# philres/ngmlr

Measured on AMD Instinct MI355X. Metric: aligned Gbp/hour (PacBio 10kb synthetic, convex-gap SW hot path, host buffers in -> results out, CIGAR bit-exact), higher is better.
Workload: dtype f32

## Files before the change

### ngmlr_amd/csrc/cvx_kernels.hip

```cpp
#include <hip/hip_runtime.h>
#include <stdint.h>

#include "cvx_types.h"
#include "cvx_launch.h"

namespace cvx {

#define CVX_DEV __device__ __forceinline__

CVX_DEV int rot1_i(int v) {
	return __builtin_amdgcn_update_dpp(0, v, 0x13C, 0xf, 0xf, true);
}
CVX_DEV float rot1_f(float v) {
	return __int_as_float(rot1_i(__float_as_int(v)));
}


CVX_DEV void row_span(const int2 ol, int W, int y, int &gs, int &ge) {
	long long lo = ol.x > 0 ? ol.x : 0;
	long long hi = (long long) ol.x + (long long) ol.y;
	if (hi > W) hi = W;
	if (hi < lo) hi = lo;
	gs = (int) (lo + y);
	ge = (int) (hi + y);
// ... 848 lines not shown
		for (int j = 0; j < M; ++j) { d[2 * j] = sh ? accA[j] << sh : accA[j]; d[2 * j + 1] = sh ? accB[j] << sh : accB[j]; }
	}

	float b = -1.0f;
	int by = 0x7fffffff, bx = 0x7fffffff;
#pragma unroll
	for (int j = 0; j < M; ++j) {
		int vy = s_besty[j][tid];
		const int ycur = (int) (ref_base - (xa[j] - (unsigned) r - 4u));
		if (ycur < H && best_r[j] >= r - cnt[j]) vy = ycur;
		const float v = best[j];
		const int vx = best_r[j] - vy;
		if (v > 0.0f) {
			if (v > b || (v == b && (vy < by || (vy == by && vx < bx)))) { b = v; by = vy; bx = vx; }
		}
	}
	float be = lbest;
#pragma unroll
	for (int off = 32; off >= 1; off >>= 1) {
		const float ob = __shfl_xor(b, off, 64);
		const int oy = __shfl_xor(by, off, 64);
		const int ox = __shfl_xor(bx, off, 64);
		if (ob > b || (ob == b && (oy < by || (oy == by && ox < bx)))) { b = ob; by = oy; bx = ox; }
		if (!EXACT) be = fmaxf(be, __shfl_xor(be, off, 64));
	}
	if (CHAIN) {
		if (lane == 0) {
			ChainOut co;
			co.score = b;
			co.best_y = (b > -1.0f) ? by + y0 : 0;
			co.best_x = (b > -1.0f) ? bx - y0 : 0;
			co.failed = chain_failed;
			a.chain_out[ct.blk] = co;
			unsigned long long *ticks = reinterpret_cast<unsigned long long *>(a.redo_count + kCtrChainTicks);
			atomicAdd(ticks, (unsigned long long) (__builtin_amdgcn_s_memtime() - chain_t0));
			if (chain_polled) atomicAdd(ticks + 1, (unsigned long long) chain_polled);
		}
		return;
	}
	if (GANG) {
		if (lane == 0) {
			s_gred[wv][0] = b; s_gred[wv][1] = __int_as_float(by); s_gred[wv][2] = __int_as_float(bx);
			s_gred[wv][3] = EXACT ? 0.0f : be;
			s_gfail[wv] = gang_failed;
		}
		__syncthreads();
		if (wv != 0) return;
#pragma unroll
		for (int w = 1; w < G; ++w) {
			const float ob = s_gred[w][0];
			const int oy = __float_as_int(s_gred[w][1]), ox = __float_as_int(s_gred[w][2]);
			if (ob > b || (ob == b && (oy < by || (oy == by && ox < bx)))) { b = ob; by = oy; bx = ox; }
			if (!EXACT) be = fmaxf(be, s_gred[w][3]);
		}
	}
	if (lane == 0) {
		TileOut o;
		o.score = b;
		o.status = 0;
		o.best_x = (b > -1.0f) ? bx : 0;
		o.best_y = (b > -1.0f) ? by : 0;
		o.ref_position = 0; o.qstart = 0; o.qend = 0; o.n_ops = 0; o.ops_first = 0;
		o.pad = (!EXACT && gswitch > 0 && !(b > be + 2.0f * a.sp.mat + 1.0f)) ? kPadRedo : 0;
		if (GANG) {
			bool failed = gang_failed != 0;
			for (int w = 1; w < G; ++w) failed = failed || s_gfail[w] != 0;
			if (failed) { o.status = -1; o.pad = 0; }
		}
		a.tout[t] = o;
	}
}

CVX_DEV int rec_load(const void *rec, const int n_dwords, const int lane) {
	return lane < n_dwords ? reinterpret_cast<const int *>(rec)[lane] : 0;
}
CVX_DEV int fld(const int w, const int k) { return __builtin_amdgcn_readlane(w, k); }
CVX_DEV unsigned long long fld64(const int w, const int k) {
	return ((unsigned long long) (unsigned) fld(w, k + 1) << 32) | (unsigned) fld(w, k);
}

CVX_DEV void walk_tile(const BacktrackArgs &a, const int t, const int lane) {
	static_assert(sizeof(TileRun) == 48 && sizeof(TileIn) == 32 && sizeof(TileOut) == 40, "record layout");
	const int wr = rec_load(a.trun + t, 12, lane);
	const int wo = rec_load(a.tout + t, 10, lane);
	if (fld(wr, 8) != 0) return;
	TileOut o;
	o.score = __int_as_float(fld(wo, 0));
	o.status = fld(wo, 1);
	o.best_x = fld(wo, 2); o.best_y = fld(wo, 3);
	o.ref_position = 0; o.qstart = 0; o.qend = 0; o.n_ops = 0; o.ops_first = 0;
	o.pad = fld(wo, 9);
	if (o.status != 0 || o.pad != 0) return;
	const int wi = rec_load(a.tin + t, 8, lane);
	const int H = fld(wi, 3), W = fld(wi, 2);
	const RowView rows = row_view(a.rsrc[t], a.rows, fld64(wi, 4));
	if (!(o.score > 0.0f)) {
		int fy, fx;
		first_cell(rows, H, W, lane, &fy, &fx);
		if (fy < 0) {
			o.score = -1.0f; o.status = 5; o.pad = 1;
			if (lane == 0) a.tout[t] = o;
			return;
		}
		o.score = 0.0f; o.best_x = fx; o.best_y = fy;
	}
	const int cb0 = fld(wr, 10);
	if (cb0 >= 0)
		backtrack_walk<true>(lane, H, fld(wr, 4), fld(wr, 6), fld(wr, 5), rows,
				reinterpret_cast<const uint2 *>(a.dirs), a.chain_blk + cb0,
				a.seq + (unsigned) fld(wi, 0), a.seq + (unsigned) fld(wi, 1),
				a.ops + fld64(wr, 2), o);
	else
		backtrack_walk<false>(lane, H, fld(wr, 4), fld(wr, 6), fld(wr, 5), rows,
				reinterpret_cast<const uint2 *>(a.dirs + fld64(wr, 0)), nullptr,
				a.seq + (unsigned) fld(wi, 0), a.seq + (unsigned) fld(wi, 1),
				a.ops + fld64(wr, 2), o);
	o.pad = 1;
	if (lane == 0) a.tout[t] = o;
}


template <int G>
struct Group {
	int gl;
	int base;
	CVX_DEV unsigned ballot(bool p) const {
		const u64 b = __builtin_amdgcn_ballot_w64(p);
		return (unsigned) (b >> base) & (G == 32 ? 0xffffffffu : ((1u << (G & 31)) - 1u));
	}
	CVX_DEV int bcast(int v, int l) const { return __shfl(v, base + l, 64); }
};

template <int G>
CVX_DEV void backtrack_walk_grp(const Group<G> g, const bool has_tile, const bool chained, const int H, const int N, const int r0, const int ops_cap,
		const RowView &rows, const uint2 *dirs, const ChainBlk *blk, const uint8_t *ref, const uint8_t *qry, int *ops, TileOut &o) {
	const int gl = g.gl;
	const int best_x = o.best_x, best_y = o.best_y;
	bool act = has_tile;
	if (has_tile && best_y <= 0) { o.status = 1; act = false; }
	const bool walked = act;

	const int qend = (H - best_y) - 1;
	int idx = ops_cap - 1;
	int elem = 4;
	int elem_len = qend;
	int consumed = qend;
	int x = best_x, y = best_y;
	int s = act ? y % N : 0;
	int status = 0;
	unsigned want = 3u;
	int budget = 2 * (best_x + best_y) + 8;

	auto emit = [&](int cur, int n) {
		if (n <= 0) return;
		if (cur == elem) {
			elem_len += n;
		} else {
			if (elem != 4) { if (gl == 0) ops[idx] = (elem_len << 4) | elem; idx -= 1; }
			elem = cur;
			elem_len = n;
		}
	};
	int c_gb = -1;
	ChainBlk c_cb;
	c_cb.dir_off = 0; c_cb.tblk0 = 0; c_cb.nblk32 = 1;

	while (__builtin_amdgcn_ballot_w64(act) != 0ull) {
		if (act) {
			bool go_on = true;
			if (--budget < 0) { status = 3; go_on = false; }
			else {
				const int dx = (want != 1u) ? 1 : 0, dy = (want != 2u) ? 1 : 0;
				const int cx = x - gl * dx, cy = y - gl * dy;
				const bool inside = (cx >= 0 && cy >= 0);
				const int lx = cx > 0 ? cx : 0, ly = cy > 0 ? cy : 0;
				int sl = s - gl * dy;
				if (sl < 0) sl += N;
				const int tt = cx + cy - r0;
				const int ttc = tt > 0 ? tt : 0;
				const RowDesc2 ol = row_at(rows, ly);
				size_t widx = (size_t) (ttc >> 5) * N + sl;
				if (chained) {
					const int gb = ly / N;
					if (gb != c_gb) { c_cb = blk[gb]; c_gb = gb; }
					int wr = (ttc >> 5) - c_cb.tblk0;
					wr = wr < 0 ? 0 : (wr >= c_cb.nblk32 ? c_cb.nblk32 - 1 : wr);
					widx = c_cb.dir_off + (size_t) wr * N + (size_t) (ly - gb * N);
				}
				const uint2 w = dirs[widx];
				const int rc = ref[lx], qc = qry[ly];
				const unsigned eqm = g.ballot(rc == qc);
				const bool in_row = inside && tt >= 0 && cx >= ol.x && cx < ol.x + ol.y;
				unsigned code = plane_code(w.x, w.y, 31 - (ttc & 31));
				if (!in_row) code = 0u;
				int minC, maxC;
				valid_bounds(ol.x, ol.y, minC, maxC);

				const unsigned full = (G == 32) ? 0xffffffffu : ((1u << (G & 31)) - 1u);
				const unsigned run = g.ballot(code == want);
				const int L = (run == full) ? G : __builtin_ctz(~run);
				const unsigned low = (L == G) ? full : ((1u << L) - 1u);
				const unsigned vp = g.ballot(cx > minC && cx < maxC);
				if ((~vp & low) != 0u) { status = 2; go_on = false; }
				else {
					if (want == 3u) {
						if (L > 0) {
							const unsigned e = eqm & low;
							const unsigned starts = (((e ^ (e << 1)) & low) & ~1u) | 1u;
							const int k = __builtin_popcount(starts);
							const int op0 = (e & 1u) ? 7 : 8;
							if (k == 1) {
								emit(op0, L);
							} else {
								const unsigned after0 = starts & ~1u;
								int len0 = __builtin_ctz(after0);
								int w0 = 0;
								if (op0 == elem) len0 += elem_len;
								else if (elem != 4) { if (gl == 0) ops[idx] = (elem_len << 4) | elem; w0 = 1; }
								const bool is_start = gl < L && ((starts >> gl) & 1u) != 0u;
								const int j = __builtin_popcount(starts & ((1u << gl) - 1u));
								const unsigned rest = (starts >> gl) >> 1;
								int mylen = rest ? __builtin_ctz(rest) + 1 : L - gl;
								if (gl == 0) mylen = len0;
								const int myop = ((e >> gl) & 1u) ? 7 : 8;
								if (is_start && j < k - 1) ops[idx - w0 - j] = (mylen << 4) | myop;
								idx -= w0 + (k - 1);
								const int lastpos = 31 - __builtin_clz(starts);
								elem = ((e >> lastpos) & 1u) ? 7 : 8;
								elem_len = L - lastpos;
							}
						}
						x -= L; y -= L; consumed += L;
					} else if (want == 1u) {
						emit(1, L);
						y -= L; consumed += L;
					} else {
						emit(2, L);
						x -= L;
					}
					if (want != 2u) { s -= L; if (s < 0) s += N; }
					if (L < G) {
						const unsigned nxt = (unsigned) g.bcast((int) code, L);
						if (nxt == 0u) go_on = false;
						else if (want != 3u) want = nxt;
						else {
							const int tp = x + y - r0;
							if (nxt == 2u) {
								const unsigned wx = (unsigned) g.bcast((int) w.x, L);
								const unsigned wy = (unsigned) g.bcast((int) w.y, L);
								const int row_lo = max(g.bcast(ol.x, L), 0);
								const int b0 = 31 - (tp & 31);
								const unsigned dm = (wx & ~wy) >> b0;
								int Ld = (~dm == 0u) ? 32 : __builtin_ctz(~dm);
								const int in_word = 32 - b0;
								const int in_rowc = x - row_lo + 1;
								if (Ld > in_rowc) Ld = in_rowc;
								const int rminC = g.bcast(minC, L), rmaxC = g.bcast(maxC, L);
								if (!(x - (Ld - 1) > rminC && x < rmaxC)) { status = 2; go_on = false; }
								else {
									emit(2, Ld);
									x -= Ld;
									if (Ld == in_rowc) go_on = false;
									else if (Ld == in_word) want = 2u;
									else {
										const unsigned c2 = plane_code(wx, wy, b0 + Ld);
										if (c2 == 0u) go_on = false; else want = c2;
									}
								}
							} else {
								const int k = gl - L;
								const int tn = tp - k;
								const bool have = (k >= 0) && (cy >= 0) && (tn >= 0) && ((tn >> 5) == (ttc >> 5));
								const bool col_in = (x >= ol.x) && (x < ol.x + ol.y);
								unsigned c2 = plane_code(w.x, w.y, 31 - (tn & 31));
								if (!col_in) c2 = 0u;
								const unsigned im = g.ballot(have && c2 == 1u) >> L;
								const int Li = (~im == 0u) ? 32 : __builtin_ctz(~im);
								const unsigned ilow = (Li >= 32) ? 0xffffffffu : ((1u << Li) - 1u);
								const unsigned vpi = g.ballot(x > minC && x < maxC) >> L;
								if ((~vpi & ilow) != 0u) { status = 2; go_on = false; }
								else {
									emit(1, Li);
									y -= Li; consumed += Li;
									s -= Li; if (s < 0) s += N;
									const int en = L + Li;
									want = 1u;
									const unsigned hv = g.ballot(have);
									const int c3i = g.bcast((int) c2, en < G ? en : 0);
									if (en < G && ((hv >> en) & 1u) != 0u) {
										if (c3i == 0) go_on = false; else want = (unsigned) c3i;
									}
								}
							}
						}
					}
				}
			}
			if (!go_on) act = false;
		}
	}
	if (walked) {
		if (status == 0) {
			if (elem != 4) { if (gl == 0) ops[idx] = (elem_len << 4) | elem; idx -= 1; }
			consumed += (y + 1);
			o.ref_position = x + 1;
			o.qstart = y + 1;
			o.qend = qend;
			o.ops_first = idx + 1;
			o.n_ops = ops_cap - 1 - idx;
			if (H != consumed) status = 3;
		}
		o.status = status;
	}
}

template <int G>
__global__ void __launch_bounds__(64)
backtrack_grp_kernel(const BacktrackArgs a, const int32_t *order, const int n_order) {
	const int lane = threadIdx.x;
	Group<G> g;
	g.gl = lane & (G - 1);
	g.base = lane & ~(G - 1);
	const int q = blockIdx.x * (64 / G) + lane / G;
	bool has = q < n_order;
	const int t = has ? order[q] : 0;
	TileOut o;
	o.score = -1.0f; o.status = 0; o.best_x = 0; o.best_y = 0;
	o.ref_position = 0; o.qstart = 0; o.qend = 0; o.n_ops = 0; o.ops_first = 0; o.pad = 0;
	TileRun tr;
	TileIn ti;
	tr.skip = 1; tr.ring = 64; tr.r0 = 0; tr.ops_cap = 8; tr.dir_off = 0; tr.ops_off = 0; tr.chain_blk0 = -1;
	ti.H = 0; ti.W = 0; ti.row_off = 0; ti.ref_off = 0; ti.qry_off = 0;
	if (has) {
		tr = a.trun[t];
		o = a.tout[t];
		ti = a.tin[t];
		if (tr.skip != 0 || o.status != 0 || o.pad != 0) has = false;
	}
	const int H = ti.H, W = ti.W;
	const RowView rows = row_view(a.rsrc[t], a.rows, ti.row_off);
	bool dead = false;
	if (__builtin_amdgcn_ballot_w64(has && !(o.score > 0.0f)) != 0ull) {
		if (has && !(o.score > 0.0f)) {
			int fy = -1, fx = 0;
			bool searching = true;
			for (int y0 = 0; __builtin_amdgcn_ballot_w64(searching && y0 < H) != 0ull; y0 += G) {
				if (searching && y0 < H) {
					const int yy = y0 + g.gl;
					bool hc = false;
					int lo_i = 0;
					if (yy < H) {
						const RowDesc2 ol = row_at(rows, yy);
						long long lo = ol.x > 0 ? ol.x : 0;
						long long hi = (long long) ol.x + (long long) ol.y;
						if (hi > W) hi = W;
						hc = hi > lo;
						lo_i = (int) lo;
					}
					const unsigned m = g.ballot(hc);
					const int l = m ? __builtin_ctz(m) : 0;
					const int fxl = g.bcast(lo_i, l);
					if (m != 0u) { fy = y0 + l; fx = fxl; searching = false; }
				}
			}
			if (fy < 0) { dead = true; has = false; }
			else { o.score = 0.0f; o.best_x = fx; o.best_y = fy; }
		}
	}
	const bool chained = tr.chain_blk0 >= 0;
	int *ops = a.ops + tr.ops_off;
	const uint8_t *ref = a.seq + ti.ref_off, *qry = a.seq + ti.qry_off;
	const uint2 *dirs = reinterpret_cast<const uint2 *>(chained ? a.dirs : a.dirs + tr.dir_off);
	backtrack_walk_grp<G>(g, has, chained, H, tr.ring, tr.r0, tr.ops_cap, rows, dirs,
			a.chain_blk + (chained ? tr.chain_blk0 : 0), ref, qry, ops, o);
	if (dead) { o.score = -1.0f; o.status = 5; }
	if ((has || dead) && g.gl == 0) { o.pad = 1; a.tout[t] = o; }
}

__global__ void __launch_bounds__(64)
backtrack_kernel(const BacktrackArgs a, const int32_t *order, const int n_order) {
	if ((int) blockIdx.x >= n_order) return;
	const int t = order ? order[blockIdx.x] : (int) blockIdx.x;
	walk_tile(a, t, threadIdx.x);
}

__global__ void __launch_bounds__(256)
finalize_kernel(const TileOut *tout, const TilePlan *plan, uint64_t *dst_off, ResultRec *res,
		BatchSummary *sum, int32_t *counters, int n_tiles, unsigned long long dense_cap) {
	constexpr int T = 256;
	__shared__ unsigned long long s_part[T];
	const int tid = threadIdx.x;
	const int per = (n_tiles + T - 1) / T;
	const int t0 = min(n_tiles, tid * per), t1 = min(n_tiles, t0 + per);
	unsigned long long mine = 0;
	for (int t = t0; t < t1; ++t) {
		const TileOut o = tout[t];
		if (o.status == 0 && o.n_ops > 0) mine += (unsigned long long) o.n_ops;
	}
	s_part[tid] = mine;
	__syncthreads();
	for (int d = 1; d < T; d <<= 1) {
		const unsigned long long v = (tid >= d) ? s_part[tid - d] : 0ull;
		__syncthreads();
		s_part[tid] += v;
		__syncthreads();
	}
	unsigned long long off = s_part[tid] - mine;
	int n_valid = 0;
	for (int t = t0; t < t1; ++t) {
		const TileOut o = tout[t];
		ResultRec r;
		r.score = o.score;
		r.status = o.status;
		r.best_x = o.best_x; r.best_y = o.best_y;
		r.ref_position = o.ref_position; r.qstart = o.qstart; r.qend = o.qend;
		r.n_ops = (o.status == 0) ? o.n_ops : 0;
		r.ops_begin = off;
		r.cells = plan[t].cells;
		res[t] = r;
		dst_off[t] = off;
		if (o.status == 0) { n_valid += 1; if (o.n_ops > 0) off += (unsigned long long) o.n_ops; }
	}
	__shared__ int s_valid;
	if (tid == 0) s_valid = 0;
	__syncthreads();
	if (n_valid) atomicAdd(&s_valid, n_valid);
	__syncthreads();
	if (tid == T - 1) {
		BatchSummary b;
		b.ops_total = s_part[T - 1];
		b.dense_cap = dense_cap;
		b.n_valid = s_valid;
		b.n_redone = counters ? counters[0] : 0;
		b.chain_task_ticks = counters ? reinterpret_cast<const unsigned long long *>(counters + kCtrChainTicks)[0] : 0ull;
		b.chain_poll_ticks = counters ? reinterpret_cast<const unsigned long long *>(counters + kCtrChainTicks)[1] : 0ull;
		*sum = b;
	}
	__syncthreads();
	if (counters && tid < 64) counters[tid] = 0;
}

__global__ void __launch_bounds__(256)
compact_ops_kernel(const int32_t *regions, const TileRun *trun, const TileOut *tout,
		const uint64_t *dst_off, uint32_t *dense, int n_tiles, unsigned long long dense_cap) {
	const int t = blockIdx.x;
	if (t >= n_tiles) return;
	const TileOut o = tout[t];
	if (o.status != 0 || o.n_ops <= 0) return;
	const unsigned long long d0 = dst_off[t];
	if (d0 + (unsigned long long) o.n_ops > dense_cap) return;
	const int32_t *src = regions + trun[t].ops_off + o.ops_first;
	uint32_t *dst = dense + d0;
	for (int i = threadIdx.x; i < o.n_ops; i += blockDim.x) dst[i] = (uint32_t) src[i];
}


__global__ void __launch_bounds__(64)
chain_reduce_kernel(const int32_t *tiles, int n_tiles, const TileRun *trun, const ChainOut *cout, TileOut *tout) {
	const int q = blockIdx.x;
	if (q >= n_tiles) return;
	const int t = tiles[q];
	const TileRun tr = trun[t];
	const int lane = threadIdx.x;
	float b = -1.0f;
	int by = 0x7fffffff, bx = 0x7fffffff, failed = 0;
	for (int g = lane; g < tr.chain_nblk; g += 64) {
		const ChainOut c = cout[tr.chain_blk0 + g];
		failed |= c.failed;
		if (c.score > b) { b = c.score; by = c.best_y; bx = c.best_x; }
	}
#pragma unroll
	for (int off = 32; off >= 1; off >>= 1) {
		const float ob = __shfl_xor(b, off, 64);
		const int oy = __shfl_xor(by, off, 64);
		const int ox = __shfl_xor(bx, off, 64);
		failed |= __shfl_xor(failed, off, 64);
		if (ob > b || (ob == b && (oy < by || (oy == by && ox < bx)))) { b = ob; by = oy; bx = ox; }
	}
	if (lane == 0) {
		TileOut o;
		o.score = b;
		o.status = failed ? -1 : 0;
		o.best_x = (b > -1.0f) ? bx : 0;
		o.best_y = (b > -1.0f) ? by : 0;
		o.ref_position = 0; o.qstart = 0; o.qend = 0; o.n_ops = 0; o.ops_first = 0;
		o.pad = 0;
		tout[t] = o;
	}
}

template <int G>
static hipError_t launch_fill_gang(const FillArgs &a, int mode, hipStream_t st) {
	if (mode == kFillExact) hipLaunchKernelGGL((fill_ring_kernel<3, false, kFillExact, false, G>), dim3(a.list_n), dim3(64 * G), 0, st, a);
	else if (a.pen_table) hipLaunchKernelGGL((fill_ring_kernel<3, false, kFillTwoPhase, true, G>), dim3(a.list_n), dim3(64 * G), 0, st, a);
	else hipLaunchKernelGGL((fill_ring_kernel<3, false, kFillTwoPhase, false, G>), dim3(a.list_n), dim3(64 * G), 0, st, a);
	return hipGetLastError();
}

template <int M, bool WRAP>
static hipError_t launch_fill_t(const FillArgs &a, int mode, size_t pad_lds, hipStream_t st) {
	if (mode == kFillChain) {
		if constexpr (M == 1 || M == 2 || M == 4) hipLaunchKernelGGL((fill_ring_kernel<M, WRAP, kFillChain>), dim3(a.list_n), dim3(64), pad_lds, st, a);
		else return hipErrorInvalidValue;
	} else if (mode == kFillExact) hipLaunchKernelGGL((fill_ring_kernel<M, WRAP, kFillExact>), dim3(a.list_n), dim3(64), 0, st, a);
	else if (!WRAP && a.pen_table) hipLaunchKernelGGL((fill_ring_kernel<M, false, kFillTwoPhase, true>), dim3(a.list_n), dim3(64), 0, st, a);
	else hipLaunchKernelGGL((fill_ring_kernel<M, WRAP, kFillTwoPhase>), dim3(a.list_n), dim3(64), 0, st, a);
	return hipGetLastError();
}

template <int M>
static hipError_t launch_fill_w(const FillArgs &a, bool wrap, int mode, size_t pad_lds, hipStream_t st) {
	return wrap ? launch_fill_t<M, true>(a, mode, pad_lds, st) : launch_fill_t<M, false>(a, mode, pad_lds, st);
}

hipError_t launch_fill(int m, int gang, bool wrap, int mode, const FillArgs &a, size_t pad_lds, hipStream_t st) {
	if (a.list_n <= 0) return hipSuccess;
	if (gang > 1) {
		if (m != 3 || wrap || mode == kFillChain) return hipErrorInvalidValue;
		return gang == 2 ? launch_fill_gang<2>(a, mode, st) : gang == 3 ? launch_fill_gang<3>(a, mode, st) : hipErrorInvalidValue;
	}
	switch (m) {
	case 1: return launch_fill_w<1>(a, wrap, mode, pad_lds, st);
	case 2: return launch_fill_w<2>(a, wrap, mode, pad_lds, st);
	case 3: return launch_fill_w<3>(a, wrap, mode, pad_lds, st);
	case 4: return launch_fill_w<4>(a, wrap, mode, pad_lds, st);
	default: return hipErrorInvalidValue;
	}
}

hipError_t launch_chain_reduce(const int32_t *tiles, int n_tiles, const TileRun *trun, const ChainOut *cout, TileOut *tout, hipStream_t st) {
	if (n_tiles <= 0) return hipSuccess;
	hipLaunchKernelGGL(chain_reduce_kernel, dim3(n_tiles), dim3(64), 0, st, tiles, n_tiles, trun, cout, tout);
	return hipGetLastError();
}

hipError_t launch_expand_rows(const RowSrc *rsrc, const TileIn *tin, const uint8_t *delta, const RowDesc *rowsx, RowDesc *rows,
		int n_tiles, bool closed_forms, hipStream_t st) {
	if (n_tiles <= 0) return hipSuccess;
	hipLaunchKernelGGL(expand_rows_kernel, dim3(n_tiles), dim3(64), 0, st, rsrc, tin, delta,
			reinterpret_cast<const int2 *>(rowsx), reinterpret_cast<int2 *>(rows), n_tiles, closed_forms ? 1 : 0);
	return hipGetLastError();
}

hipError_t launch_plan(const RowDesc *rows, const RowSrc *rsrc, const TileIn *tin, TilePlan *plan, int n_tiles, uint64_t rows_per_tile,
		unsigned long long max_matrix_mb, hipStream_t st) {
	if (n_tiles <= 0) return hipSuccess;
	if (rows_per_tile >= 1024)
		hipLaunchKernelGGL(plan_kernel<256>, dim3(n_tiles), dim3(256), 0, st,
				reinterpret_cast<const int2 *>(rows), rsrc, tin, plan, n_tiles, max_matrix_mb);
	else
		hipLaunchKernelGGL(plan_kernel<64>, dim3((n_tiles + 3) / 4), dim3(256), 0, st,
				reinterpret_cast<const int2 *>(rows), rsrc, tin, plan, n_tiles, max_matrix_mb);
	return hipGetLastError();
}

hipError_t launch_backtrack(const BacktrackArgs &a, const int32_t *order, int n_order, int group, hipStream_t st) {
	if (a.n_tiles <= 0) return hipSuccess;
	if (group == 16 && order != nullptr) {
		if (n_order <= 0) return hipSuccess;
		hipLaunchKernelGGL(backtrack_grp_kernel<16>, dim3((n_order + 3) / 4), dim3(64), 0, st, a, order, n_order);
	} else if (group == 4 && order != nullptr) {
		if (n_order <= 0) return hipSuccess;
		hipLaunchKernelGGL(backtrack_grp_kernel<4>, dim3((n_order + 15) / 16), dim3(64), 0, st, a, order, n_order);
	} else if (group == 8 && order != nullptr) {
		if (n_order <= 0) return hipSuccess;
		hipLaunchKernelGGL(backtrack_grp_kernel<8>, dim3((n_order + 7) / 8), dim3(64), 0, st, a, order, n_order);
	} else if (group == 32 && order != nullptr) {
		if (n_order <= 0) return hipSuccess;
		hipLaunchKernelGGL(backtrack_grp_kernel<32>, dim3((n_order + 1) / 2), dim3(64), 0, st, a, order, n_order);
	} else {
		const int nb = order != nullptr ? n_order : a.n_tiles;
		if (nb <= 0) return hipSuccess;
		hipLaunchKernelGGL(backtrack_kernel, dim3(nb), dim3(64), 0, st, a, order, nb);
	}
	return hipGetLastError();
}

hipError_t launch_finalize(const TileOut *tout, const TilePlan *plan, uint64_t *dst_off, ResultRec *res,
		BatchSummary *sum, int32_t *counters, int n_tiles, uint64_t dense_cap, hipStream_t st) {
	hipLaunchKernelGGL(finalize_kernel, dim3(1), dim3(256), 0, st, tout, plan, dst_off, res, sum, counters,
			n_tiles, (unsigned long long) dense_cap);
	return hipGetLastError();
}

hipError_t launch_compact(const int32_t *regions, const TileRun *trun, const TileOut *tout,
		const uint64_t *dst_off, uint32_t *dense, int n_tiles, uint64_t dense_cap, hipStream_t st) {
	if (n_tiles <= 0) return hipSuccess;
	hipLaunchKernelGGL(compact_ops_kernel, dim3(n_tiles), dim3(256), 0, st, regions, trun, tout, dst_off, dense, n_tiles,
			(unsigned long long) dense_cap);
	return hipGetLastError();
}

}
```

### ngmlr_amd/csrc/cvx_launch.h

```cpp
#ifndef CVX_LAUNCH_H
#define CVX_LAUNCH_H

#include <hip/hip_runtime_api.h>
#include <stdint.h>

#include "cvx_types.h"

namespace cvx {

hipError_t launch_fill(int m, int gang, bool wrap, int mode, const FillArgs &a, size_t pad_lds, hipStream_t st);
hipError_t launch_chain_reduce(const int32_t *tiles, int n_tiles, const TileRun *trun, const ChainOut *cout, TileOut *tout, hipStream_t st);
struct ScorePair {
	uint64_t ref_off, qry_off;
	uint64_t scratch_off;
	int32_t ref_len, qry_len;
};
hipError_t launch_score(const uint8_t *seq, const ScorePair *pairs, int32_t *scratch, float *out, int n, int max_ref_len, hipStream_t st);
hipError_t launch_score_diag(const uint8_t *seq, const ScorePair *pairs, float *out, int n, hipStream_t st);

struct SearchCandidate {
	uint64_t location;
	float score;
	int32_t reverse;
};
struct SearchArgs {
	const uint2 *rows;
	const uint32_t *locs;
	unsigned long long unit_offset;
	int32_t k;
	const uint8_t *seq;
	const uint64_t *seq_off;
	const int32_t *seq_len;
	int32_t n;
	unsigned long long *events;
	const uint64_t *list_off;
	uint32_t *rlist;
	uint32_t *undo;
	SearchCandidate *cand;
	int32_t *n_cand;
	float *max_hit;
	int32_t *kmer_misses;
	const int32_t *work;
	int32_t n_work;
	int32_t bits;
	float hpoc_factor;
	uint64_t *keys;
	float *scores;
	float sensitivity, min_hits;
	int32_t bin_shift;
	const uint64_t *cand_off;
};
static const int kSearchWaveLog2Min = 9, kSearchWaveLog2Max = 12, kSearchWaveLog2Default = 11;
static const int kSearchWaveSeq = 4096;
static inline int search_wave_entries(const int log2s) { return (3 << log2s) / 4; }
static inline int search_wave_log2(const unsigned long long votes) {
	for (int l = kSearchWaveLog2Min; l < kSearchWaveLog2Max; ++l) if (votes <= (unsigned long long) search_wave_entries(l)) return l;
	return kSearchWaveLog2Max;
}
static const int kSearchNeedsHbm = -2;
size_t search_wave_lds_bytes(int log2s, int seq_cap, bool slot8);
hipError_t launch_search_count(const SearchArgs &a, hipStream_t st);
hipError_t launch_search(const SearchArgs &a, hipStream_t st);
hipError_t launch_search_wave(const SearchArgs &a, int log2s, int seq_cap, bool slot8, hipStream_t st);
hipError_t launch_search_wave_hbm(const SearchArgs &a, int n_tables, unsigned int *ticket, hipStream_t st);
hipError_t launch_search_compact(const SearchCandidate *sparse, const uint64_t *src_off, const int32_t *n_cand, const uint64_t *dst_begin,
		SearchCandidate *dense, int n, hipStream_t st);

hipError_t launch_decode_windows(const uint8_t *bin, const uint64_t *starts, int n_starts,
		const WindowDesc *win, int n, uint8_t *dst, hipStream_t st);

hipError_t launch_text_size(const TextArgs &a, hipStream_t st);
hipError_t launch_text_write(const TextArgs &a, hipStream_t st);
hipError_t launch_nm_offsets(const TextArgs &a, int first, int count, unsigned long long *len, unsigned long long *off, unsigned long long *total, hipStream_t st);
hipError_t launch_nm_profile(const TextArgs &a, int first, int count, const unsigned long long *off, int32_t *triples, hipStream_t st);

size_t generic_scratch_bytes(int ring);
hipError_t launch_fill_generic(const FillArgs &a, bool sse_variant, uint8_t *scratch, const uint64_t *scratch_off, hipStream_t st);
hipError_t launch_expand_rows(const RowSrc *rsrc, const TileIn *tin, const uint8_t *delta, const RowDesc *rowsx, RowDesc *rows,
		int n_tiles, bool closed_forms, hipStream_t st);
hipError_t launch_plan(const RowDesc *rows, const RowSrc *rsrc, const TileIn *tin, TilePlan *plan, int n_tiles, uint64_t rows_per_tile,
		unsigned long long max_matrix_mb, hipStream_t st);
hipError_t launch_backtrack(const BacktrackArgs &a, const int32_t *order, int n_order, int group, hipStream_t st);
hipError_t launch_finalize(const TileOut *tout, const TilePlan *plan, uint64_t *dst_off, ResultRec *res,
		BatchSummary *sum, int32_t *counters, int n_tiles, uint64_t dense_cap, hipStream_t st);
hipError_t launch_compact(const int32_t *regions, const TileRun *trun, const TileOut *tout,
		const uint64_t *dst_off, uint32_t *dense, int n_tiles, uint64_t dense_cap, hipStream_t st);

}
#endif
```

### ngmlr_amd/csrc/cvx_rt_align.cpp

```cpp
#include <algorithm>
#include <atomic>
#include <chrono>
#include <cstdio>
#include <cstdlib>
#include <cstring>
#include <new>
#include <string>
#include <vector>

#include "cvx_rt.h"

namespace {

static const size_t kPoolBatches = 8;

cvx_batch_s *acquire_batch(cvx_context *h) {
	if (!h->pool.empty()) {
		cvx_batch_s *b = h->pool.back();
		h->pool.pop_back();
		return b;
	}
	return new (std::nothrow) cvx_batch_s();
}

void recycle_batch(cvx_context *h, cvx_batch_s *b) {
	const bool failed = b->state == kFailed;
	b->state = kEmpty;
	b->in_flight = false;
	b->have_ops = false;
	b->have_refs = false;
	b->text_done = false;
	b->fail_rc = CVX_OK;
	b->fail_msg.clear();
	if (h) {
		auto it = std::find(h->live.begin(), h->live.end(), b);
		if (it != h->live.end()) h->live.erase(it);
	}
	if (h && !failed && h->pool.size() < kPoolBatches) { h->pool.push_back(b); return; }
	b->release();
	delete b;
}

void discard_batch(cvx_context *h, cvx_batch_s *b) {
	(void) hipDeviceSynchronize();
	if (h) {
		auto it = std::find(h->pending.begin(), h->pending.end(), b);
		if (it != h->pending.end()) h->pending.erase(it);
		it = std::find(h->live.begin(), h->live.end(), b);
		if (it != h->live.end()) h->live.erase(it);
	}
	b->release();
	delete b;
}

int fail_job(cvx_batch_s *b, int rc) {
	(void) hipDeviceSynchronize();
	b->state = kFailed;
	b->fail_rc = rc;
	b->fail_msg = g_err;
	return rc;
}

int stage_upload(cvx_context *h, cvx_batch_s *b, int32_t n, const cvx_tile *tiles,
		const cvx_genome_s *genome = nullptr, const uint64_t *ref_position = nullptr) {
	RC_TRY(ensure_streams(h));
	UploadLayout L;
	std::vector<TileIn> tin;
	int bad = -1;
	const bool windows = genome != nullptr;
	const int lrc = upload_layout(n, tiles, tin, L, &bad, windows);
	if (lrc == kLayoutMalformed) { set_err("tile %d malformed", bad); return CVX_ERR_ARG; }
	if (lrc == kLayoutTooLarge) {
		set_err("%llu sequence bytes exceed one batch (4 GiB); split the batch", (unsigned long long) L.seq_total);
		return CVX_ERR_ARG;
	}
	b->n = n;
	b->state = kEmpty;
	b->have_ops = false;
	b->have_refs = false;
	b->text_done = false;
	b->ops_total = 0;
	b->seq_total = L.seq_total;
	b->n_rows = L.n_rows;
	memset(&b->timing, 0, sizeof(b->timing));
	RC_TRY(b->make_events());
	const size_t n1 = (size_t) std::max(n, 1);
	const size_t rows1 = (size_t) std::max<uint64_t>(L.arena_rows, 1);
	RC_TRY(b->h_delta.ensure((size_t) L.delta_total + 256));
	RC_TRY(b->h_rsrc.ensure(n1 * sizeof(RowSrc)));
	RC_TRY(b->d_delta.ensure((size_t) L.delta_total + 256));
	RC_TRY(b->d_rsrc.ensure(n1));
	RC_TRY(b->h_tin.ensure(n1 * sizeof(TileIn)));
	RC_TRY(b->h_plan.ensure(n1 * sizeof(TilePlan)));
	RC_TRY(b->h_res.ensure(n1 * sizeof(ResultRec) + sizeof(BatchSummary)));
	RC_TRY(b->d_seq.ensure((size_t) L.seq_total + 256));
	RC_TRY(b->d_rows.ensure(rows1));
	RC_TRY(b->d_tin.ensure(n1));
	RC_TRY(b->d_plan.ensure(n1));
	RC_TRY(b->d_trun.ensure(n1));
	RC_TRY(b->d_tout.ensure(n1));
	RC_TRY(b->d_dstoff.ensure(n1));
	RC_TRY(b->d_lists.ensure(2 * n1));
	if (b->d_counters.cap < 64) {
		RC_TRY(b->d_counters.ensure(64));
		HIP_TRY(hipMemset(b->d_counters.p, 0, b->d_counters.cap * sizeof(int32_t)));
	}
	RC_TRY(b->d_res.ensure(n1 * sizeof(ResultRec) + sizeof(BatchSummary)));
	if (n) memcpy(b->h_tin.p, tin.data(), (size_t) n * sizeof(TileIn));

	const bool zc_qry = n > 0 && L.qry_contig && L.qry_bytes > 0 && in_pinned_block(tiles[0].qry, L.qry_bytes + 4);
	const bool zc_ref = n > 0 && !windows && L.ref_contig && L.ref_bytes > 0 && in_pinned_block(tiles[0].ref, L.ref_bytes + 4);
	b->zero_copy_bytes = (zc_qry ? L.qry_bytes : 0) + (zc_ref ? L.ref_bytes : 0);
	const bool pack_seq = !(zc_qry && (zc_ref || windows));
	if (pack_seq) RC_TRY(b->h_seq.ensure((size_t) L.seq_total + 256));
	uint8_t *hseq = b->h_seq.as<uint8_t>();
	uint8_t *hdelta = b->h_delta.as<uint8_t>();
	std::vector<RowOverflow> overflow;
	hipStream_t st = h->s_io;
	if (pack_seq) upload_zero_pads(L, hseq);
	if (zc_qry || zc_ref) {
		const uint64_t zmax = L.pad + 1024;
		RC_TRY(b->h_zero.ensure((size_t) zmax));
		if (b->zero_cap != b->h_zero.cap) { memset(b->h_zero.p, 0, b->h_zero.cap); b->zero_cap = b->h_zero.cap; }
		auto zero_range = [&](uint64_t lo, uint64_t hi) -> int {
			lo = lo / 256 * 256;
			hi = std::min<uint64_t>((hi + 255) / 256 * 256, (L.seq_total + 255) / 256 * 256);
			for (uint64_t at = lo; at < hi; at += zmax / 256 * 256) {
				const uint64_t len = std::min<uint64_t>(hi - at, zmax / 256 * 256);
				HIP_TRY(hipMemcpyAsync(b->d_seq.p + at, b->h_zero.p, (size_t) len, hipMemcpyHostToDevice, st));
			}
			return CVX_OK;
		};
		if (zc_qry) {
			RC_TRY(zero_range(0, L.qry_base));
			RC_TRY(zero_range(L.qry_base + L.qry_bytes, L.ref_base));
			HIP_TRY(hipMemcpyAsync(b->d_seq.p + L.qry_base, tiles[0].qry, (size_t) ((L.qry_bytes + 3) / 4 * 4), hipMemcpyHostToDevice, st));
		}
		if (zc_ref) {
			RC_TRY(zero_range(L.ref_base + L.ref_bytes, L.seq_total));
			HIP_TRY(hipMemcpyAsync(b->d_seq.p + L.ref_base, tiles[0].ref, (size_t) ((L.ref_bytes + 3) / 4 * 4), hipMemcpyHostToDevice, st));
		}
	}
	uint64_t pack_work = L.delta_total * 9ull;
	if (!zc_qry) pack_work += L.qry_bytes;
	if (!zc_ref && !windows) pack_work += L.ref_bytes;
	const std::vector<uint64_t> &wprefix = L.wprefix;
	int threads = std::max(1, std::min(h->pack_threads, PackPool::get().size()));
	if (pack_work < (8u << 20)) threads = 1;
	const int pieces = threads > 1 ? 8 : 1;
	int t0 = 0;
	uint64_t a_done = 0, b_done = L.ref_base, delta_done = 0;
	const uint64_t a_end_all = L.ref_base, b_end_all = (L.seq_total + 255) / 256 * 256;
	for (int pc = 1; pc <= pieces; ++pc) {
		int t1 = n;
		if (pc < pieces) {
			const uint64_t target = wprefix[(size_t) n] / (uint64_t) pieces * (uint64_t) pc;
			t1 = (int) (std::upper_bound(wprefix.begin(), wprefix.end(), target) - wprefix.begin());
			t1 = std::min(std::max(t1, t0), n);
		}
		if (t1 > t0 && pack_work > 0) {
			std::vector<uint64_t> wp((size_t) (t1 - t0) + 1);
			for (int i = t0; i <= t1; ++i) wp[(size_t) (i - t0)] = wprefix[(size_t) i] - wprefix[(size_t) t0];
			const int base = t0;
			const size_t first = overflow.size();
			overflow.resize(first + (size_t) threads + 1);
			std::atomic<int> slot(0);
			parallel_ranges(t1 - t0, wp, threads, [&](int bg, int en) {
				upload_pack(base + bg, base + en, tiles, tin, hseq, hdelta, L.rsrc, overflow[first + (size_t) slot.fetch_add(1)], !zc_qry, !zc_ref && !windows);
			});
		}
		if (!zc_qry) {
			const uint64_t a_end = (t1 == n) ? a_end_all : (uint64_t) tin[(size_t) t1].qry_off / 256 * 256;
			if (a_end > a_done) HIP_TRY(hipMemcpyAsync(b->d_seq.p + a_done, hseq + a_done, (size_t) (a_end - a_done), hipMemcpyHostToDevice, st));
			a_done = std::max(a_done, a_end);
		}
		if (!zc_ref && !windows) {
			const uint64_t b_end = (t1 == n) ? b_end_all : (uint64_t) tin[(size_t) t1].ref_off / 256 * 256;
			if (b_end > b_done) HIP_TRY(hipMemcpyAsync(b->d_seq.p + b_done, hseq + b_done, (size_t) (b_end - b_done), hipMemcpyHostToDevice, st));
			b_done = std::max(b_done, b_end);
		}
		if (L.delta_total) {
			uint64_t del_end = L.delta_total;
			if (t1 < n) {
				int q = t1;
				while (q < n && L.rsrc[(size_t) q].fmt != kRowsDelta8 && L.rsrc[(size_t) q].fmt != kRowsExplicit) q++;
				if (q < n) del_end = L.rsrc[(size_t) q].src_off;
			}
			del_end = (t1 == n) ? (del_end + 255) / 256 * 256 : del_end / 256 * 256;
			if (del_end > delta_done)
				HIP_TRY(hipMemcpyAsync(b->d_delta.p + delta_done, hdelta + delta_done, (size_t) (del_end - delta_done), hipMemcpyHostToDevice, st));
			delta_done = std::max(delta_done, del_end);
		}
		t0 = t1;
	}
	if (n) HIP_TRY(hipMemcpyAsync(b->d_tin.p, b->h_tin.p, (size_t) n * sizeof(TileIn), hipMemcpyHostToDevice, st));
	if (n) {
		uint64_t n_x = 0;
		for (const RowOverflow &o : overflow) n_x += o.rows.size();
		b->n_rowsx = n_x;
		if (n_x) {
			RC_TRY(b->h_rowsx.ensure((size_t) n_x * sizeof(RowDesc)));
			RC_TRY(b->d_rowsx.ensure((size_t) n_x));
			RowDesc *hx = b->h_rowsx.as<RowDesc>();
			uint64_t at = 0;
			for (const RowOverflow &o : overflow) {
				uint64_t r = 0;
				for (int32_t ti : o.tiles) {
					L.rsrc[(size_t) ti].src_off = at + r;
					r += (uint64_t) tin[(size_t) ti].H;
				}
				if (!o.rows.empty()) memcpy(hx + at, o.rows.data(), o.rows.size() * sizeof(RowDesc));
				at += o.rows.size();
			}
			HIP_TRY(hipMemcpyAsync(b->d_rowsx.p, hx, (size_t) n_x * sizeof(RowDesc), hipMemcpyHostToDevice, st));
		}
		memcpy(b->h_rsrc.p, L.rsrc.data(), (size_t) n * sizeof(RowSrc));
		HIP_TRY(hipMemcpyAsync(b->d_rsrc.p, b->h_rsrc.p, (size_t) n * sizeof(RowSrc), hipMemcpyHostToDevice, st));
		if (L.arena_rows) HIP_TRY(launch_expand_rows(b->d_rsrc.p, b->d_tin.p, b->d_delta.p, b->d_rowsx.p, b->d_rows.p, n, false, st));
	}
	if (windows && n) {
		RC_TRY(b->h_win.ensure((size_t) n * sizeof(WindowDesc)));
		RC_TRY(b->d_win.ensure((size_t) n));
		WindowDesc *hw = b->h_win.as<WindowDesc>();
		for (int i = 0; i < n; ++i) {
			hw[i].position = ref_position[i];
			hw[i].dst_off = tin[(size_t) i].ref_off;
			hw[i].n_chars = tiles[i].ref_len;
		}
		HIP_TRY(hipMemcpyAsync(b->d_win.p, hw, (size_t) n * sizeof(WindowDesc), hipMemcpyHostToDevice, st));
		HIP_TRY(hipMemsetAsync(b->d_seq.p + L.ref_base + L.ref_bytes, 0, (size_t) (L.seq_total - L.ref_base - L.ref_bytes), st));
		HIP_TRY(launch_decode_windows(genome->d_bin.p, genome->d_starts.p, genome->n_starts, b->d_win.p, n, b->d_seq.p, st));
		RC_TRY(b->h_refs.ensure((size_t) L.ref_bytes + 64));
		HIP_TRY(hipMemcpyAsync(b->h_refs.p, b->d_seq.p + L.ref_base, (size_t) L.ref_bytes, hipMemcpyDeviceToHost, st));
		b->refs_base = L.ref_base;
		b->have_refs = true;
	}
	b->state = kUploaded;
	return CVX_OK;
}

int stage_plan(cvx_context *h, cvx_batch_s *b, hipStream_t st) {
	const int n = b->n;
	HIP_TRY(hipEventRecord(b->ev[0], st));
	if (n) {
		HIP_TRY(launch_plan(b->d_rows.p, b->d_rsrc.p, b->d_tin.p, b->d_plan.p, n, b->n_rows / (uint64_t) n, h->max_matrix_mb, st));
		HIP_TRY(hipMemcpyAsync(b->h_plan.p, b->d_plan.p, (size_t) n * sizeof(TilePlan), hipMemcpyDeviceToHost, st));
	}
	HIP_TRY(hipEventRecord(b->ev[1], st));
	HIP_TRY(hipEventRecord(b->ev_in, st));
	b->state = kPlanned;
	return CVX_OK;
}

int stage_compute(cvx_context *h, cvx_batch_s *b, bool streaming = false) {
// ... 702 lines not shown
```

Measured before the change: 16060.

## Branchless backtrack walk, waves-per-EU hint, and multi-block finalize scan

The backtrack walk loop is restructured so the bounds check is folded into the run ballot, emit becomes branchless, and the gap step is merged into a single deferred position update, which reduces divergence and ballots per step. The backtrack kernel gets an amdgpu_waves_per_eu(6) hint that trades registers for occupancy. The single-block finalize kernel is replaced by a two-pass multi-block prefix sum: per-block partials are stored after dst_off, then each block scans its own tiles. This costs an extra launch and a larger dst_off buffer, and the register cap could cause spills.

```diff
diff --git a/ngmlr_amd/csrc/cvx_kernels.hip b/ngmlr_amd/csrc/cvx_kernels.hip
--- a/ngmlr_amd/csrc/cvx_kernels.hip
+++ b/ngmlr_amd/csrc/cvx_kernels.hip
@@ -1024,24 +1024,24 @@
 	int budget = 2 * (best_x + best_y) + 8;
 
 	auto emit = [&](int cur, int n) {
-		if (n <= 0) return;
-		if (cur == elem) {
-			elem_len += n;
-		} else {
-			if (elem != 4) { if (gl == 0) ops[idx] = (elem_len << 4) | elem; idx -= 1; }
-			elem = cur;
-			elem_len = n;
-		}
+		const bool some = n > 0;
+		const bool same = cur == elem;
+		const bool flush = some && !same && elem != 4;
+		if (flush && gl == 0) ops[idx] = (elem_len << 4) | elem;
+		idx -= flush ? 1 : 0;
+		elem_len = some ? (same ? elem_len + n : n) : elem_len;
+		elem = some ? cur : elem;
 	};
 	int c_gb = -1;
 	ChainBlk c_cb;
 	c_cb.dir_off = 0; c_cb.tblk0 = 0; c_cb.nblk32 = 1;
 
-	while (__builtin_amdgcn_ballot_w64(act) != 0ull) {
+	if (__builtin_amdgcn_ballot_w64(act) != 0ull) do {
 		if (act) {
-			bool go_on = true;
-			if (--budget < 0) { status = 3; go_on = false; }
-			else {
+			const bool spent = --budget < 0;
+			bool go_on = !spent;
+			if (spent) status = 3;
+			{
 				const int dx = (want != 1u) ? 1 : 0, dy = (want != 2u) ? 1 : 0;
 				const int cx = x - gl * dx, cy = y - gl * dy;
 				const bool inside = (cx >= 0 && cy >= 0);
@@ -1069,54 +1069,45 @@
 				valid_bounds(ol.x, ol.y, minC, maxC);
 
 				const unsigned full = (G == 32) ? 0xffffffffu : ((1u << (G & 31)) - 1u);
-				const unsigned run = g.ballot(code == want);
-				const int L = (run == full) ? G : __builtin_ctz(~run);
+				const unsigned run = g.ballot(code == want && cx > minC && cx < maxC);
+				const int Lr = (run == full) ? G : __builtin_ctz(~run);
+				const unsigned nxt = (unsigned) g.bcast((int) code, Lr & (G - 1));
+				const bool rejected = !spent && Lr < G && nxt == want;
+				if (rejected) { status = 2; go_on = false; }
+				const int L = go_on ? Lr : 0;
 				const unsigned low = (L == G) ? full : ((1u << L) - 1u);
-				const unsigned vp = g.ballot(cx > minC && cx < maxC);
-				if ((~vp & low) != 0u) { status = 2; go_on = false; }
-				else {
-					if (want == 3u) {
-						if (L > 0) {
-							const unsigned e = eqm & low;
-							const unsigned starts = (((e ^ (e << 1)) & low) & ~1u) | 1u;
+				{
+					int gap_op = 0, gap_n = 0;
+					const int mx0 = (want != 1u) ? L : 0, my0 = (want != 2u) ? L : 0;
+					int mx = mx0, my = my0;
+					unsigned nwant = want;
+					{
+						const bool diag = want == 3u;
+						const unsigned e = eqm & low;
+						const unsigned starts = (((e ^ (e << 1)) & low) & ~1u) | 1u;
+						const unsigned after0 = diag ? (starts & ~1u) : 0u;
+						emit(diag ? ((e & 1u) ? 7 : 8) : (int) want, (L > 0 && after0 != 0u) ? __builtin_ctz(after0) : L);
+						if (L > 0 && after0 != 0u) {
 							const int k = __builtin_popcount(starts);
-							const int op0 = (e & 1u) ? 7 : 8;
-							if (k == 1) {
-								emit(op0, L);
-							} else {
-								const unsigned after0 = starts & ~1u;
-								int len0 = __builtin_ctz(after0);
-								int w0 = 0;
-								if (op0 == elem) len0 += elem_len;
-								else if (elem != 4) { if (gl == 0) ops[idx] = (elem_len << 4) | elem; w0 = 1; }
-								const bool is_start = gl < L && ((starts >> gl) & 1u) != 0u;
-								const int j = __builtin_popcount(starts & ((1u << gl) - 1u));
-								const unsigned rest = (starts >> gl) >> 1;
-								int mylen = rest ? __builtin_ctz(rest) + 1 : L - gl;
-								if (gl == 0) mylen = len0;
-								const int myop = ((e >> gl) & 1u) ? 7 : 8;
-								if (is_start && j < k - 1) ops[idx - w0 - j] = (mylen << 4) | myop;
-								idx -= w0 + (k - 1);
-								const int lastpos = 31 - __builtin_clz(starts);
-								elem = ((e >> lastpos) & 1u) ? 7 : 8;
-								elem_len = L - lastpos;
-							}
+							const bool is_start = gl < L && ((starts >> gl) & 1u) != 0u;
+							const int j = __builtin_popcount(starts & ((1u << gl) - 1u));
+							const unsigned rest = (starts >> gl) >> 1;
+							int mylen = rest ? __builtin_ctz(rest) + 1 : L - gl;
+							if (gl == 0) mylen = elem_len;
+							const int myop = ((e >> gl) & 1u) ? 7 : 8;
+							if (is_start && j < k - 1) ops[idx - j] = (mylen << 4) | myop;
+							idx -= k - 1;
+							const int lastpos = 31 - __builtin_clz(starts);
+							elem = ((e >> lastpos) & 1u) ? 7 : 8;
+							elem_len = L - lastpos;
 						}
-						x -= L; y -= L; consumed += L;
-					} else if (want == 1u) {
-						emit(1, L);
-						y -= L; consumed += L;
-					} else {
-						emit(2, L);
-						x -= L;
 					}
-					if (want != 2u) { s -= L; if (s < 0) s += N; }
-					if (L < G) {
-						const unsigned nxt = (unsigned) g.bcast((int) code, L);
+					if (go_on && L < G) {
 						if (nxt == 0u) go_on = false;
-						else if (want != 3u) want = nxt;
+						else if (want != 3u) nwant = nxt;
 						else {
-							const int tp = x + y - r0;
+							const int xg = x - mx0, yg = y - my0;
+							const int tp = xg + yg - r0;
 							if (nxt == 2u) {
 								const unsigned wx = (unsigned) g.bcast((int) w.x, L);
 								const unsigned wy = (unsigned) g.bcast((int) w.y, L);
@@ -1125,52 +1116,55 @@
 								const unsigned dm = (wx & ~wy) >> b0;
 								int Ld = (~dm == 0u) ? 32 : __builtin_ctz(~dm);
 								const int in_word = 32 - b0;
-								const int in_rowc = x - row_lo + 1;
+								const int in_rowc = xg - row_lo + 1;
 								if (Ld > in_rowc) Ld = in_rowc;
 								const int rminC = g.bcast(minC, L), rmaxC = g.bcast(maxC, L);
-								if (!(x - (Ld - 1) > rminC && x < rmaxC)) { status = 2; go_on = false; }
+								if (!(xg - (Ld - 1) > rminC && xg < rmaxC)) { status = 2; go_on = false; }
 								else {
-									emit(2, Ld);
-									x -= Ld;
+									gap_op = 2; gap_n = Ld;
+									mx += Ld;
 									if (Ld == in_rowc) go_on = false;
-									else if (Ld == in_word) want = 2u;
+									else if (Ld == in_word) nwant = 2u;
 									else {
 										const unsigned c2 = plane_code(wx, wy, b0 + Ld);
-										if (c2 == 0u) go_on = false; else want = c2;
+										if (c2 == 0u) go_on = false; else nwant = c2;
 									}
 								}
 							} else {
 								const int k = gl - L;
 								const int tn = tp - k;
 								const bool have = (k >= 0) && (cy >= 0) && (tn >= 0) && ((tn >> 5) == (ttc >> 5));
-								const bool col_in = (x >= ol.x) && (x < ol.x + ol.y);
+								const bool col_in = (xg >= ol.x) && (xg < ol.x + ol.y);
 								unsigned c2 = plane_code(w.x, w.y, 31 - (tn & 31));
 								if (!col_in) c2 = 0u;
 								const unsigned im = g.ballot(have && c2 == 1u) >> L;
 								const int Li = (~im == 0u) ? 32 : __builtin_ctz(~im);
 								const unsigned ilow = (Li >= 32) ? 0xffffffffu : ((1u << Li) - 1u);
-								const unsigned vpi = g.ballot(x > minC && x < maxC) >> L;
+								const unsigned vpi = g.ballot(xg > minC && xg < maxC) >> L;
 								if ((~vpi & ilow) != 0u) { status = 2; go_on = false; }
 								else {
-									emit(1, Li);
-									y -= Li; consumed += Li;
-									s -= Li; if (s < 0) s += N;
+									gap_op = 1; gap_n = Li;
+									my += Li;
 									const int en = L + Li;
-									want = 1u;
+									nwant = 1u;
 									const unsigned hv = g.ballot(have);
 									const int c3i = g.bcast((int) c2, en < G ? en : 0);
 									if (en < G && ((hv >> en) & 1u) != 0u) {
-										if (c3i == 0) go_on = false; else want = (unsigned) c3i;
+										if (c3i == 0) go_on = false; else nwant = (unsigned) c3i;
 									}
 								}
 							}
 						}
+						emit(gap_op, gap_n);
 					}
+					x -= mx; y -= my; consumed += my;
+					s -= my; if (s < 0) s += N;
+					want = nwant;
 				}
 			}
 			if (!go_on) act = false;
 		}
-	}
+	} while (__builtin_amdgcn_ballot_w64(act) != 0ull);
 	if (walked) {
 		if (status == 0) {
 			if (elem != 4) { if (gl == 0) ops[idx] = (elem_len << 4) | elem; idx -= 1; }
@@ -1187,7 +1181,7 @@
 }
 
 template <int G>
-__global__ void __launch_bounds__(64)
+__global__ void __launch_bounds__(64) __attribute__((amdgpu_waves_per_eu(6)))
 backtrack_grp_kernel(const BacktrackArgs a, const int32_t *order, const int n_order) {
 	const int lane = threadIdx.x;
 	Group<G> g;
@@ -1256,19 +1250,50 @@
 	walk_tile(a, t, threadIdx.x);
 }
 
-__global__ void __launch_bounds__(256)
-finalize_kernel(const TileOut *tout, const TilePlan *plan, uint64_t *dst_off, ResultRec *res,
+constexpr int kFinalizeThreads = 256;
+
+CVX_DEV unsigned long long block_sum(unsigned long long v, unsigned long long *s_w, const int tid) {
+#pragma unroll
+	for (int off = 32; off >= 1; off >>= 1) v += __shfl_xor(v, off, 64);
+	__syncthreads();
+	if ((tid & 63) == 0) s_w[tid >> 6] = v;
+	__syncthreads();
+	return s_w[0] + s_w[1] + s_w[2] + s_w[3];
+}
+
+__global__ void __launch_bounds__(kFinalizeThreads)
+finalize_sums_kernel(const TileOut *tout, unsigned long long *part, int n_tiles) {
+	__shared__ unsigned long long s_w[kFinalizeThreads / 64];
+	const int tid = threadIdx.x;
+	const int t = blockIdx.x * kFinalizeThreads + tid;
+	unsigned long long mine = 0, valid = 0;
+	if (t < n_tiles) {
+		const TileOut o = tout[t];
+		if (o.status == 0) { valid = 1; if (o.n_ops > 0) mine = (unsigned long long) o.n_ops; }
+	}
+	const unsigned long long ops = block_sum(mine, s_w, tid);
+	const unsigned long long nv = block_sum(valid, s_w, tid);
+	if (tid == 0) { part[2 * blockIdx.x] = ops; part[2 * blockIdx.x + 1] = nv; }
+}
+
+__global__ void __launch_bounds__(kFinalizeThreads)
+finalize_kernel(const TileOut *tout, const TilePlan *plan, uint64_t *dst_off, const unsigned long long *part, ResultRec *res,
 		BatchSummary *sum, int32_t *counters, int n_tiles, unsigned long long dense_cap) {
-	constexpr int T = 256;
+	constexpr int T = kFinalizeThreads;
+	__shared__ unsigned long long s_w[T / 64];
 	__shared__ unsigned long long s_part[T];
 	const int tid = threadIdx.x;
-	const int per = (n_tiles + T - 1) / T;
-	const int t0 = min(n_tiles, tid * per), t1 = min(n_tiles, t0 + per);
-	unsigned long long mine = 0;
-	for (int t = t0; t < t1; ++t) {
-		const TileOut o = tout[t];
-		if (o.status == 0 && o.n_ops > 0) mine += (unsigned long long) o.n_ops;
-	}
+	const int blk = blockIdx.x, n_blk = gridDim.x;
+	const int upto = blk == 0 ? n_blk : blk;
+	unsigned long long before = 0, valid_all = 0;
+	for (int j = tid; j < upto; j += T) { before += part[2 * j]; valid_all += part[2 * j + 1]; }
+	before = block_sum(before, s_w, tid);
+	if (blk == 0) valid_all = block_sum(valid_all, s_w, tid);
+	const int t = blk * T + tid;
+	TileOut o;
+	o.status = -1; o.n_ops = 0;
+	if (t < n_tiles) o = tout[t];
+	const unsigned long long mine = (o.status == 0 && o.n_ops > 0) ? (unsigned long long) o.n_ops : 0ull;
 	s_part[tid] = mine;
 	__syncthreads();
 	for (int d = 1; d < T; d <<= 1) {
@@ -1277,10 +1302,8 @@
 		s_part[tid] += v;
 		__syncthreads();
 	}
-	unsigned long long off = s_part[tid] - mine;
-	int n_valid = 0;
-	for (int t = t0; t < t1; ++t) {
-		const TileOut o = tout[t];
+	if (t < n_tiles) {
+		const unsigned long long off = (blk == 0 ? 0ull : before) + s_part[tid] - mine;
 		ResultRec r;
 		r.score = o.score;
 		r.status = o.status;
@@ -1291,18 +1314,13 @@
 		r.cells = plan[t].cells;
 		res[t] = r;
 		dst_off[t] = off;
-		if (o.status == 0) { n_valid += 1; if (o.n_ops > 0) off += (unsigned long long) o.n_ops; }
-	}
-	__shared__ int s_valid;
-	if (tid == 0) s_valid = 0;
-	__syncthreads();
-	if (n_valid) atomicAdd(&s_valid, n_valid);
-	__syncthreads();
+	}
+	if (blk != 0) return;
 	if (tid == T - 1) {
 		BatchSummary b;
-		b.ops_total = s_part[T - 1];
+		b.ops_total = before;
 		b.dense_cap = dense_cap;
-		b.n_valid = s_valid;
+		b.n_valid = (int32_t) valid_all;
 		b.n_redone = counters ? counters[0] : 0;
 		b.chain_task_ticks = counters ? reinterpret_cast<const unsigned long long *>(counters + kCtrChainTicks)[0] : 0ull;
 		b.chain_poll_ticks = counters ? reinterpret_cast<const unsigned long long *>(counters + kCtrChainTicks)[1] : 0ull;
@@ -1450,7 +1468,10 @@
 
 hipError_t launch_finalize(const TileOut *tout, const TilePlan *plan, uint64_t *dst_off, ResultRec *res,
 		BatchSummary *sum, int32_t *counters, int n_tiles, uint64_t dense_cap, hipStream_t st) {
-	hipLaunchKernelGGL(finalize_kernel, dim3(1), dim3(256), 0, st, tout, plan, dst_off, res, sum, counters,
+	const int n_blk = n_tiles > 0 ? (n_tiles + kFinalizeThreads - 1) / kFinalizeThreads : 1;
+	unsigned long long *part = reinterpret_cast<unsigned long long *>(dst_off) + (n_tiles > 0 ? n_tiles : 0);
+	hipLaunchKernelGGL(finalize_sums_kernel, dim3(n_blk), dim3(kFinalizeThreads), 0, st, tout, part, n_tiles);
+	hipLaunchKernelGGL(finalize_kernel, dim3(n_blk), dim3(kFinalizeThreads), 0, st, tout, plan, dst_off, part, res, sum, counters,
 			n_tiles, (unsigned long long) dense_cap);
 	return hipGetLastError();
 }
diff --git a/ngmlr_amd/csrc/cvx_launch.h b/ngmlr_amd/csrc/cvx_launch.h
--- a/ngmlr_amd/csrc/cvx_launch.h
+++ b/ngmlr_amd/csrc/cvx_launch.h
@@ -2,6 +2,7 @@
 #define CVX_LAUNCH_H
 
 #include <hip/hip_runtime_api.h>
+#include <stddef.h>
 #include <stdint.h>
 
 #include "cvx_types.h"
@@ -81,6 +82,7 @@
 hipError_t launch_plan(const RowDesc *rows, const RowSrc *rsrc, const TileIn *tin, TilePlan *plan, int n_tiles, uint64_t rows_per_tile,
 		unsigned long long max_matrix_mb, hipStream_t st);
 hipError_t launch_backtrack(const BacktrackArgs &a, const int32_t *order, int n_order, int group, hipStream_t st);
+inline size_t finalize_words(size_t n_tiles) { return n_tiles + 2 * ((n_tiles + 255) / 256) + 2; }
 hipError_t launch_finalize(const TileOut *tout, const TilePlan *plan, uint64_t *dst_off, ResultRec *res,
 		BatchSummary *sum, int32_t *counters, int n_tiles, uint64_t dense_cap, hipStream_t st);
 hipError_t launch_compact(const int32_t *regions, const TileRun *trun, const TileOut *tout,
diff --git a/ngmlr_amd/csrc/cvx_rt_align.cpp b/ngmlr_amd/csrc/cvx_rt_align.cpp
--- a/ngmlr_amd/csrc/cvx_rt_align.cpp
+++ b/ngmlr_amd/csrc/cvx_rt_align.cpp
@@ -99,7 +99,7 @@
 	RC_TRY(b->d_plan.ensure(n1));
 	RC_TRY(b->d_trun.ensure(n1));
 	RC_TRY(b->d_tout.ensure(n1));
-	RC_TRY(b->d_dstoff.ensure(n1));
+	RC_TRY(b->d_dstoff.ensure(finalize_words(n1)));
 	RC_TRY(b->d_lists.ensure(2 * n1));
 	if (b->d_counters.cap < 64) {
 		RC_TRY(b->d_counters.ensure(64));
```

Measured after the change: 16210 (median of 6 runs). About the same (+0.9%).
